# zwu88/TANTE

Measured on AMD Instinct MI355X. Metric: rollout frames/sec (fwd), TANTE on 256x256 Active Matter, higher is better.
Workload: dtype bf16

## Files before the change

### tante_amd/_lib.py

```python
import ctypes as C
import os

HERE = os.path.dirname(os.path.abspath(__file__))
LIB_PATH = os.environ.get("TANTE_LIB") or os.path.join(HERE, "lib", "libtante_hip.so")

F32, BF16 = 0, 1
ACT_NONE, ACT_GELU_ERF, ACT_GELU_TANH, ACT_RELU = 0, 1, 2, 3
A_LINEAR, A_PATCH_NHWC, A_PATCH_NCHW = 0, 1, 2
E_LINEAR, E_FILM, E_DECONV_NHWC, E_DECONV_NCHW = 0, 1, 2, 3
W_LINEAR, W_CONV_NHWC, W_DECONV_NHWC, W_DECONV_NCHW = 0, 1, 2, 3
W_LINEAR_T, W_CONV_NHWC_T, W_DECONV_NHWC_T, W_DECONV_NCHW_T = 4, 5, 6, 7

c_i32, c_i64, c_f32, c_vp = C.c_int32, C.c_int64, C.c_float, C.c_void_p


class PackGeom(C.Structure):
    _fields_ = [("n_pad", c_i32), ("k_pad", c_i32), ("nt", c_i32), ("cb", c_i32), ("bytes", c_i64)]


class Gemm(C.Structure):
    _fields_ = [
        ("a", c_vp), ("a_dtype", c_i32), ("a_mode", c_i32), ("M", c_i32), ("K", c_i32),
        ("a_s1", c_i64), ("a_s0", c_i64), ("a_off", c_i64), ("a_n0", c_i32),
        ("Hin", c_i32), ("Win", c_i32), ("Cin", c_i32), ("P", c_i32), ("ln", c_i32), ("ln_eps", c_f32),
# ... 160 lines not shown
    "tante_layernorm_bwd": ([c_vp, c_i32, c_vp, c_vp, c_vp, c_i64, c_i32, c_vp, c_vp], c_i32),
    "tante_act_fwd": ([c_vp, c_i32, c_vp, c_i32, c_i64, c_i32, c_vp], c_i32),
    "tante_act_bwd": ([c_vp, c_i32, c_vp, c_i32, c_vp, c_i32, c_i64, c_i32, c_vp], c_i32),
    "tante_colsum": ([c_vp, c_i32, c_i64, c_i32, c_i64, c_vp, c_i32, c_vp], c_i32),
    "tante_film_pos_fwd": ([c_vp, c_vp, c_vp, c_vp, c_i64, c_i32, c_i32, c_i64, c_vp, c_vp], c_i32),
    "tante_pos_embed_tmajor": ([c_vp, c_vp, c_vp, c_i64, c_i32, c_i64, c_i32, c_vp, c_vp], c_i32),
    "tante_film_pos_bwd": ([c_vp, c_vp, c_vp, c_i64, c_i64, c_i32, c_i32, c_vp, c_vp, c_vp, c_vp, c_vp], c_i32),
    "tante_taylor_bwd": ([c_vp, c_i64, C.POINTER(c_vp), c_i32, C.c_double, c_i32, c_vp, c_i64, c_i32, c_i64, c_i64, c_vp], c_i32),
    "tante_attention_bwd": ([c_vp, c_vp, c_vp, c_i32, c_i32, c_i32, C.POINTER(Seq), c_i32, c_f32, C.c_uint64, c_vp], c_i32),
    "tante_attention_dropout": ([c_vp, c_vp, c_i32, c_i32, c_i32, C.POINTER(Seq), c_i32, c_f32, C.c_uint64, c_vp], c_i32),
    "tante_dropout_add": ([c_vp, c_i32, c_vp, c_f32, C.c_uint64, c_i64, c_vp, c_vp], c_i32),
    "tante_dropout_bwd": ([c_vp, c_f32, C.c_uint64, c_i64, c_vp, c_i32, c_vp], c_i32),
    "tante_axis_mlp_bwd": ([c_vp, c_vp, c_i64, c_i32, c_i64, c_vp, c_vp, c_vp, c_vp, c_vp, c_vp, c_vp], c_i32),
    "tante_fold_fwd": ([c_vp, c_vp, c_vp, c_vp, c_i32, c_i32, c_vp, c_vp, c_vp], c_i32),
    "tante_fold_bwd": ([c_vp, c_vp, c_vp, c_vp, c_vp, c_i32, c_i32, c_vp, c_vp, c_vp, c_vp, c_vp], c_i32),
    "tante_fold_bwd_clear": ([c_vp, c_vp, c_vp, c_vp, c_vp, c_i32, c_i32, c_vp, c_vp, c_vp, c_vp, c_vp], c_i32),
    "tante_fold_bwd_multi": ([c_vp, c_i32, c_i32, c_vp], c_i32),
    "tante_fold_fwd_multi": ([c_vp, c_i32, c_vp], c_i32),
    "tante_axis_mlp_film_supported": ([c_i64, c_i32, c_i32, c_i64, c_i32], c_i32),
    "tante_axis_mlp_film": ([c_vp, c_vp, c_vp, c_vp, c_vp, c_i64, c_i32, c_i32, c_i64, c_i32, c_vp, c_vp, c_vp, c_vp, c_vp], c_i32),
    "tante_film_pos_fwd_frames": ([c_vp, c_vp, c_vp, c_vp, c_i64, c_i32, c_i64, c_i32, c_vp, c_vp], c_i32),
    "tante_film_pos_bwd_frames": ([c_vp, c_vp, c_vp, c_i64, c_i64, c_i32, c_i32, c_vp, c_vp, c_vp, c_vp, c_vp], c_i32),
    "tante_film_pos_bwd_frames_acc": ([c_vp, c_vp, c_vp, c_i64, c_i64, c_i32, c_i32, c_vp, c_i32, c_vp, c_vp, c_vp, c_i32, c_vp], c_i32),
    "tante_film_table_bwd": ([c_vp, c_i32, c_i32] + [c_vp] * 6 + [c_vp, c_vp] + [c_vp] * 8 + [c_i32, c_vp], c_i32),
    "tante_pack_block_train_multi": ([c_vp, c_i32, c_i32, c_i32, c_vp], c_i32),
    "tante_pack_block_tail_bwd_multi": ([c_vp, c_i32, c_i32, c_i32, c_vp], c_i32),
    "tante_axis_mlp_bwd_fused_supported": ([c_i32, c_i64], c_i32),
    "tante_axis_mlp_bwd_fused": ([c_vp, c_vp, c_i64, c_i32, c_i64, c_vp, c_vp, c_vp, c_vp, c_vp, c_vp, c_vp, c_vp, c_vp], c_i32),
    "tante_axis_mlp_bwd_fused_ws": ([c_vp, c_vp, c_i64, c_i32, c_i64, c_vp, c_vp, c_vp, c_vp, c_vp, c_vp, c_vp, c_vp, c_vp, c_i64, c_vp], c_i32),
    "tante_axis_wgrad": ([c_vp, c_vp, c_i64, c_i32, c_i64, c_vp, c_vp, c_i32, c_vp], c_i32),
    "tante_axis_wgrad_workspace_bytes": ([], c_i64),
    "tante_set_seed_mix": ([c_vp], c_i32),
    "tante_axis_wgrad_ws": ([c_vp, c_vp, c_i64, c_i32, c_i64, c_vp, c_vp, c_i32, c_vp, c_i64, c_vp], c_i32),
    "tante_wgrad": ([C.POINTER(RowMat), C.POINTER(RowMat), c_i64, c_i32, c_i32, c_vp, c_vp, c_i32, c_i32, c_i32, c_i32, c_i32, c_i32, c_vp], c_i32),
    "tante_wgrad_ws": ([C.POINTER(RowMat), C.POINTER(RowMat), c_i64, c_i32, c_i32, c_vp, c_vp, c_i32, c_i32, c_i32, c_i32, c_i32, c_i32, c_vp, c_i64, c_vp], c_i32),
    "tante_wgrad_multi_ws": ([c_vp, c_vp, c_i32, c_i64, c_i32, c_i32, c_vp, c_vp, c_i32, c_i32, c_i32, c_i32, c_i32, c_i32, c_vp, c_i64, c_vp], c_i32),
    "tante_wgrad_multi": ([c_vp, c_vp, c_i32, c_i64, c_i32, c_i32, c_vp, c_vp, c_i32, c_i32, c_i32, c_i32, c_i32, c_i32, c_vp], c_i32),
    "tante_clip_value": ([c_vp, c_i64, c_f32, c_vp], c_i32),
    "tante_rt_reduce_bwd": ([c_vp, c_i32, c_i32, c_vp, c_vp], c_i32),
    "tante_last_error": ([], C.c_char_p),
    "tante_abi_version": ([], c_i32),
    "tante_set_option": ([C.c_char_p, c_i32], c_i32),
    "tante_nan_to_num": ([c_vp, c_vp, c_i64, c_vp], c_i32),
    "tante_head_fused_multi": ([c_i32, c_vp, c_vp, c_vp, c_i32, c_i64, c_i64, c_i64, c_i32, c_i32, c_i32, c_i32, c_i32, c_vp, c_i64, c_vp, c_i64,
                               c_vp], c_i32),
    "tante_head_fused_multi_streams": ([c_i32, c_vp, c_vp, c_vp, c_i32, c_i64, c_i64, c_i64, c_i32, c_i32, c_i32, c_i32, c_i32, c_vp, c_i64, c_vp, c_i64,
                               c_vp], c_i32),
    "tante_spectral_bf16out_supported": ([c_i64, c_i32, c_i32, c_i32, c_i32, c_i32, c_i32], c_i32),
    "tante_spectral_layer_bf16out": ([c_vp, c_i64, c_i32, c_i32, c_i32, c_vp, c_vp, c_i32, c_i32, c_i32, c_i32, c_vp, c_vp, c_i32, c_i32, c_vp, c_vp,
                                     c_i64, c_vp], c_i32),
    "tante_get_option": ([C.c_char_p, c_i32], c_i32),
    "tante_attention_masked": ([c_vp, c_vp, c_i32, c_i32, c_i32, c_i32, c_i32, c_i32, c_vp, c_i64, c_vp, c_vp], c_i32),
    "tante_attention_masked_bwd": ([c_vp, c_vp, c_vp, c_i32, c_i32, c_i32, c_i32, c_i32, c_i32, c_vp, c_i64, c_vp, c_vp, c_vp], c_i32),
    "tante_attention_flash_stats_floats": ([c_i32, C.POINTER(Seq)], c_i64),
    "tante_attention_flash_supported": ([c_i32, c_i32, c_i32, c_i32], c_i32),
    "tante_attention_flash": ([c_vp, c_vp, c_vp, c_i32, c_i32, c_i32, C.POINTER(Seq), c_i32, c_f32, C.c_uint64, c_vp], c_i32),
    "tante_attention_flash_bwd": ([c_vp, c_vp, c_vp, c_vp, c_vp, c_i32, c_i32, c_i32, C.POINTER(Seq), c_i32, c_f32, C.c_uint64, c_vp], c_i32),
    "tante_attention_flash_masked": ([c_vp, c_vp, c_vp, c_i32, c_i32, c_i32, c_i32, c_i32, c_i32, c_vp, c_i64, c_vp, c_f32, C.c_uint64, c_vp], c_i32),
    "tante_attention_flash_masked_bwd": ([c_vp, c_vp, c_vp, c_vp, c_vp, c_i32, c_i32, c_i32, c_i32, c_i32, c_i32, c_vp, c_i64, c_vp, c_f32, C.c_uint64, c_vp], c_i32),
    "tante_head_enc_supported": ([c_i32, c_i32], c_i32),
    "tante_head_enc_stream_bytes": ([c_i32], c_i64),
    "tante_head_enc_ws_bytes": ([c_i64], c_i64),
    "tante_pack_head_enc": ([c_vp] * 6 + [c_i32, c_i32, c_vp, c_vp], c_i32),
    "tante_head_enc_fused": ([c_i32, c_vp, c_vp, c_vp, c_i32, c_i64, c_i64, c_i64, c_i32, c_i32, c_i32, c_i32, c_i32, c_vp, c_i64, c_vp, c_i64,
                             c_vp, c_vp, c_vp, c_i64, c_vp], c_i32),
    "tante_adaptive_tail_supported": ([c_i32] * 6, c_i32),
    "tante_adaptive_rt_stream_bytes": ([c_i32], c_i64),
    "tante_adaptive_ws_bytes": ([c_i32, c_i32, c_i32, c_i32], c_i64),
    "tante_pack_adaptive_rt": ([c_vp] * 6 + [c_i32, c_vp, c_vp], c_i32),
    "tante_adaptive_rt": ([c_i32, c_vp, c_vp, c_vp, c_i32, c_i64, c_i64, c_i64, c_i32, c_i32, c_i32, c_i32, c_f32, c_f32, c_vp, c_i64,
                           c_vp, c_vp, c_vp, c_vp, c_vp, c_vp], c_i32),
    "tante_head_adaptive": ([c_i32, c_vp, c_vp, c_i32, c_i64, c_i64, c_i64, c_i32, c_i32, c_i32, c_i32, c_i32, c_vp, c_vp, c_vp, c_i32, c_vp,
                             c_i32, c_vp, c_i64, c_vp, c_i64, c_vp], c_i32),
    "tante_afno_filter_supported": ([c_i64, c_i32, c_i32, c_i32, c_i32], c_i32),
    "tante_afno_twiddle_floats": ([c_i32, c_i32], c_i64),
    "tante_afno_filter_workspace_bytes": ([c_i64, c_i32, c_i32, c_i32], c_i64),
    "tante_afno_filter": ([c_vp, c_vp, c_i64, c_i32, c_i32, c_i32, c_i32, c_vp, c_vp, c_vp, c_f32, c_vp, c_vp, c_i64, c_vp], c_i32),
}

LIB_OPTIONS = ("TANTE_ATTN_BWD_HG", "TANTE_ATTN_BWD_NO_SPLIT", "TANTE_ATTN_BWD_VALU", "TANTE_ATTN_FWD_VALU", "TANTE_AXIS_BWD_SMALL_WGS",
               "TANTE_AXIS_BLOCKS", "TANTE_AXIS_BWD_WGS", "TANTE_AXIS_CT", "TANTE_AXIS_FILM", "TANTE_AXIS_GENERIC", "TANTE_AXIS_MFMA", "TANTE_AXIS_NT", "TANTE_AXIS_WGRAD_WGS",
               "TANTE_BLOCK_KERNEL", "TANTE_COLSUM_ROWS", "TANTE_CVIT_CHAIN_TOKENS", "TANTE_ENC23_SPLIT", "TANTE_FILM_BWD_ROWS",
               "TANTE_FS_GROUPS", "TANTE_FS_HALF", "TANTE_FS_SKEW", "TANTE_FS_WAVES", "TANTE_GEMM_NO_LITE", "TANTE_GEMM_SMALLM", "TANTE_GEMM_WGS", "TANTE_HEAD_WAVES",
               "TANTE_IM2COL_TILED", "TANTE_RESIZE_TILED", "TANTE_SPECTRAL_BF16OUT", "TANTE_SPECTRAL_DFT", "TANTE_SPECTRAL_X3", "TANTE_WGRAD_DEEP",
               "TANTE_WGRAD_JOBS", "TANTE_WGRAD_JOBS_WGS", "TANTE_WGRAD_NO_SLAB", "TANTE_WGRAD_NO_TR", "TANTE_WGRAD_REDUCE_NY",
               "TANTE_WGRAD_RG", "TANTE_WGRAD_SLAB_WGS", "TANTE_WGRAD_TR_WGS", "TANTE_WGRAD_WGS", "TANTE_XATTN_GPW", "TANTE_XATTN_STREAM", "TANTE_XATTN_VALU",)


_lib = None
ABI_VERSION = 14


def lib():
    global _lib
    if _lib is None:
        if not os.path.exists(LIB_PATH):
            raise RuntimeError(
                f"{LIB_PATH} is missing: build it with `python -m tante_amd.build` "
                "(or __graft_entry__.build()).  tante_amd has no CPU / eager fallback.")
        L = C.CDLL(LIB_PATH)
        for name, (argtypes, restype) in SIGNATURES.items():
            fn = getattr(L, name)
            fn.argtypes = argtypes
            fn.restype = restype
        got = int(L.tante_abi_version())
        if got != ABI_VERSION:
            raise RuntimeError(f"{LIB_PATH}: library ABI {got}, this binding expects {ABI_VERSION} -- a stale build (or a stale variant under "
                               "TANTE_LIB); rebuild with `python -m tante_amd.build`")
        _lib = L
        import warnings
        for k in LIB_OPTIONS:
            v = os.environ.get(k)
            if v is None:
                continue
            try:
                rc = L.tante_set_option(k.encode(), int(v))
            except ValueError:
                warnings.warn(f"{k}={v!r}: library options are integers; ignored")
                continue
            if rc != 0:
                warnings.warn(f"{k}={v}: tante_set_option refused it ({L.tante_last_error().decode(errors='replace')})")
    return _lib


def set_option(name: str, value: int) -> None:
    check(lib().tante_set_option(name.encode(), int(value)), "tante_set_option")


def get_option(name: str, default: int = 0) -> int:
    return int(lib().tante_get_option(name.encode(), int(default)))


def check(rc: int, what: str = ""):
    if rc != 0:
        msg = lib().tante_last_error().decode(errors="replace")
        raise RuntimeError(f"libtante_hip {what} failed (rc={rc}): {msg}")
```

### tante_amd/csrc/block_sliced.hip

```cpp
#include "common.hip.h"
#include "fused_common.hip.h"
#include "fs_common.hip.h"
#include "block_sliced.h"

namespace {


struct FsArgs {
  float* x;
  const char* w;
  TanteSeq sq;
  int causal;
  float eps;
  int spw;
  unsigned magic;
  float* out;
  unsigned short *xh1, *qkv, *o, *xh2, *hpre, *act;
  float *st1, *x1, *st2;
  float p_drop;
  unsigned long long seed_attn, seed_out, seed_mlp;
  const unsigned long long* seed_mix;
  unsigned long long* stamps;
  const float* tprop;
  int skew;
};

#ifdef TANTE_ABLATE
#define FS_STAMP(k)                                                                                        \
  do {                                                                                                     \
    if (A.stamps) {                                                                                        \
      unsigned long long t_;                                                                               \
      __builtin_amdgcn_sched_barrier(0);                                                                   \
      asm volatile("s_memtime %0\n\ts_waitcnt lgkmcnt(0)" : "=s"(t_)::"memory");                          \
      __builtin_amdgcn_sched_barrier(0);                                                                   \
      if (lane == 0) A.stamps[((long)vblock * 8 + wave) * 20 + (k)] = t_;                               \
    }                                                                                                      \
  } while (0)
unsigned long long* g_fs_stamps = nullptr;
#else
#define FS_STAMP(k)
#endif

__device__ __forceinline__ void fs_divmod(int a, int n, float rn, int& q, int& r) {
  q = (int)((float)a * rn);
  r = a - q * n;
  if (r >= n) { ++q; r -= n; }
  if (r < 0) { --q; r += n; }
}
struct FsSeqMap {
  float rs0, rl0;
  __device__ __forceinline__ explicit FsSeqMap(const TanteSeq& q) : rs0(__builtin_amdgcn_rcpf((float)q.n_s0)), rl0(__builtin_amdgcn_rcpf((float)q.n_l0)) {}
  __device__ __forceinline__ long token(const TanteSeq& q, int s, int l) const {
    int a, b, c, d;
    fs_divmod(s, q.n_s0, rs0, a, b);
    fs_divmod(l, q.n_l0, rl0, c, d);
    return (long)a * q.S1 + (long)b * q.S0 + (long)c * q.P1 + (long)d * q.P0;
  }
};


struct TpropW {
  float w1c[4], w2c[4];
  f32x4 b1v, b2v;
};
__device__ __forceinline__ void tprop_weights(const float* __restrict__ tp, int lane, TpropW& w) {
#pragma unroll
  for (int a = 0; a < 4; ++a) { w.w1c[a] = tp[4 * (lane & 3) + a]; w.w2c[a] = tp[20 + 4 * (lane & 3) + a]; }
  w.b1v = f32x4{tp[16], tp[17], tp[18], tp[19]};
  w.b2v = f32x4{tp[36], tp[37], tp[38], tp[39]};
}
__device__ __forceinline__ void tprop_apply(const TpropW& w, f32x4 (&xs)[4]) {
  f32x4 hid[4], yy[4];
#pragma unroll
  for (int e = 0; e < 4; ++e) {
    f32x4 h = w.b1v;
#pragma unroll
    for (int a = 0; a < 4; ++a) h = __builtin_amdgcn_mfma_f32_4x4x1f32(w.w1c[a], xs[a][e], h, 0, 0, 0);
    hid[e] = h;
  }
#pragma unroll
  for (int e = 0; e < 4; ++e) hid[e] = gelu_poly4<false>(hid[e]);
#pragma unroll
  for (int e = 0; e < 4; ++e) {
    f32x4 acc = f32x4{xs[0][e], xs[1][e], xs[2][e], xs[3][e]} + w.b2v;
#pragma unroll
    for (int j = 0; j < 4; ++j) acc = __builtin_amdgcn_mfma_f32_4x4x1f32(w.w2c[j], hid[e][j], acc, 0, 0, 0);
    yy[e] = acc;
  }
#pragma unroll
  for (int t = 0; t < 4; ++t) xs[t] = f32x4{yy[0][t], yy[1][t], yy[2][t], yy[3][t]};
}

constexpr int fs_group(int ntt, int nk) {
  int g = 1;
  for (int d = 1; d <= ntt; ++d)
    if (ntt % d == 0 && d * nk <= 8) g = d;
  return g;
}

template <int TPS, int NTT, int NW, bool TRAIN, int G = 1, bool TPROP = false, bool LASTQ = false>
__global__ __launch_bounds__(64 * NW * G, 2) void block_fs_kernel(FsArgs A) {
  static_assert(!TPROP || (TPS == 1 && !TRAIN), "the fused temporal propagator: T letter (L = 4), inference");
  static_assert(!LASTQ || (TPS == 1 && NW == 4 && G == 1 && !TRAIN), "the last-slot form: T letter (L = 4), 4 waves, inference");
  static_assert(G == 1 || (G == 2 && NW == 4), "the paired form is two 4-wave groups");
  constexpr int RT = 16 / NW;
  constexpr int HPW = RT / 2;
  constexpr int FS_PF8 = 3, FS_PF4 = 2;
  constexpr bool TIGHT = (NW == 4 && NTT == 4 && (TRAIN || TPS == 0)) || (NW == 8 && NTT == 8);
  constexpr int PF = (NW == 8 ? FS_PF8 : FS_PF4) - (TIGHT ? 1 : 0);
  constexpr int IMG = 16 * NTT * FS_ROW;
  constexpr int LDS_G = 2 * IMG + 16 * NTT * NW * 8 + FS_BIAS_FLOATS * 4;
  extern __shared__ __attribute__((aligned(16))) char smem_all[];
  const int grp = G == 1 ? 0 : __builtin_amdgcn_readfirstlane((int)threadIdx.x >> 8);
  char* const smem = smem_all + grp * LDS_G;
  char* const bufA = smem;
  char* const bufB = smem + IMG;
  char* const stat = smem + 2 * IMG;
  float* const lbias = (float*)(stat + 16 * NTT * NW * 8);
  const int tid = threadIdx.x & (64 * NW - 1), lane = tid & 63, kk = lane >> 4, l15 = lane & 15;
  const int wave = __builtin_amdgcn_readfirstlane(tid >> 6);
  const int vblock = (int)blockIdx.x * G + grp;
  if constexpr (G == 2) {
    if (grp == 1) __builtin_amdgcn_s_barrier();
  }
  if constexpr (G == 1) {
    if ((__builtin_amdgcn_s_getreg(0x1804) & 1u) == 1u) __builtin_amdgcn_s_setprio(3);
  }
  if constexpr (!TRAIN && G == 1) {
    if (A.skew > 0 && blockIdx.x >= (gridDim.x >> 1)) {
      for (int i = 0; i < A.skew; ++i) __builtin_amdgcn_s_sleep(8);
    }
  }
  float* const x = A.x;
  const unsigned long long smix = (TRAIN && A.seed_mix) ? *A.seed_mix : 0ull;
  const unsigned long long sd_attn = A.seed_attn ^ smix;
  const int L = A.sq.L;
  const int seq0 = vblock * A.spw;
  const int nlive = min(A.spw, A.sq.nseq - seq0) * L;
  const int nslot = A.spw * L;

  const FsW wq = fs_wstream(A.w, (unsigned)((RT * wave) * FS_FRAG + lane * 16));
  u32x4 wb[PF + 1][RT];
  FS_STAMP(0);
#ifdef TANTE_ABLATE
  if (A.stamps && lane == 0) {
    A.stamps[((long)vblock * 8 + wave) * 20 + 16] = __builtin_amdgcn_s_getreg((31 << 11) | 4);
    A.stamps[((long)vblock * 8 + wave) * 20 + 17] = __builtin_amdgcn_s_getreg((31 << 11) | 20);
    A.stamps[((long)vblock * 8 + wave) * 20 + 18] = __builtin_amdgcn_s_memrealtime();
  }
#endif
  int tslot[2];
  {
    const FsSeqMap smap(A.sq);
#pragma unroll
    for (int h = 0; h < (16 * NTT > 64 ? 2 : 1); ++h) {
      const int slot = lane + 64 * h;
      const int s = (int)(((unsigned)slot * A.magic) >> 16), p = slot - s * L;
      tslot[h] = slot < nlive ? (int)smap.token(A.sq, seq0 + s, p) : -1;
    }
  }
  auto tok_of = [&](int slot) { return __shfl(slot < 64 ? tslot[0] : tslot[16 * NTT > 64 ? 1 : 0], slot & 63); };
  for (int i = tid; i < FS_BIAS_FLOATS / 4; i += 64 * NW) *(f32x4*)(lbias + 4 * i) = *(const f32x4*)((const float*)(A.w + FS_W_BYTES) + 4 * i);
  FS_STAMP(1);
  int tokidx[NTT];
#pragma unroll
  for (int tt = 0; tt < NTT; ++tt) tokidx[tt] = tok_of(16 * tt + l15);

  constexpr int CPR = 4 * RT, RPI = 64 / CPR, ROWB = CPR * 16, TILEB = 16 * ROWB;
  constexpr int NSUB = (IMG / NW) / TILEB >= 2 ? 2 : 1;
  static_assert((IMG / NW) >= TILEB, "staging piece too small");
  char* const stg = bufA + wave * (IMG / NW);
  const int rrow = lane / CPR, rchunk = lane % CPR;
  auto srow = [&](int j) { return RPI * j + rrow; };
  auto slice_load = [&](const float* __restrict__ src, f32x4 (&raw)[NTT][RT]) {
#pragma unroll
    for (int tt = 0; tt < NTT; ++tt)
#pragma unroll
      for (int j = 0; j < RT; ++j) {
        const int t = tok_of(16 * tt + srow(j));
        raw[tt][j] = *(const f32x4*)(src + (long)(t < 0 ? 0 : t) * FS_C + 16 * RT * wave + 4 * rchunk);
      }
  };
  auto slice_to_acc = [&](const f32x4 (&raw)[NTT][RT], f32x4 (&acc)[RT][NTT]) {
#pragma unroll
    for (int tt = 0; tt < NTT; ++tt) {
      char* sb = stg + (tt % NSUB) * TILEB;
#pragma unroll
// ... 46 lines not shown
          xv[i][t] = *(const f32x4*)(x + (long)(tk < 0 ? 0 : tk) * FS_C + 4 * lane);
        }
      fs_wring_prime<0, RT, PF>(wq, wb);
      TpropW tw;
      tprop_weights(A.tprop, lane, tw);
#pragma unroll
      for (int i = 0; i < GPW; ++i) {
        tprop_apply(tw, xv[i]);
#pragma unroll
        for (int t = 0; t < 4; ++t) {
          const f32x4 y = xv[i][t];
          const int tk = tok_of(4 * (wave * GPW + i) + t);
          const bool live = tk >= 0;
          if (live && (!LASTQ || t == 3)) *(f32x4*)(x + (long)tk * FS_C + 4 * lane) = y;
          float sm = (y[0] + y[1]) + (y[2] + y[3]);
          float sq = fmaf(y[0], y[0], fmaf(y[1], y[1], fmaf(y[2], y[2], y[3] * y[3])));
          sm = rows_sum(row16_sum(sm));
          sq = rows_sum(row16_sum(sq));
          const float mean = sm * (1.0f / FS_C);
          const float var = fmaxf(sq * (1.0f / FS_C) - mean * mean, 0.0f);
          const float rstd = live ? rsqrtf(var + A.eps) : 0.0f;
          const float sh = live ? -mean * rstd : 0.0f;
          const int slot = 4 * (wave * GPW + i) + t;
          u32x2 o2;
          o2[0] = pack_bf16x2(fmaf(y[0], rstd, sh), fmaf(y[1], rstd, sh));
          o2[1] = pack_bf16x2(fmaf(y[2], rstd, sh), fmaf(y[3], rstd, sh));
          *(u32x2*)(bufA + slot * FS_ROW + (((lane >> 1) ^ (slot & 15)) << 4) + (lane & 1) * 8) = o2;
        }
      }
    }
  }
  if constexpr (!ln1_done) {
    constexpr int GPW = 4 * NTT / NW;
    static_assert(GPW * NW == 4 * NTT, "token rows must split evenly over the waves");
    f32x4 v[GPW][4];
    bool lv[GPW];
    int tis[GPW];
#pragma unroll
    for (int i = 0; i < GPW; ++i) {
      const int ti = tis[i] = tok_of(4 * (wave * GPW + i) + kk);
      lv[i] = ti >= 0;
      const float* row = x + (long)(lv[i] ? ti : 0) * FS_C;
#pragma unroll
      for (int j = 0; j < 4; ++j) v[i][j] = *(const f32x4*)(row + 4 * (l15 + 16 * j));
    }
    fs_wring_prime<0, RT, PF>(wq, wb);
#pragma unroll
    for (int i = 0; i < GPW; ++i) {
      float s = 0.f, q = 0.f;
#pragma unroll
      for (int j = 0; j < 4; ++j)
#pragma unroll
        for (int e = 0; e < 4; ++e) {
          s += v[i][j][e];
          q = fmaf(v[i][j][e], v[i][j][e], q);
        }
      s = row16_sum(s);
      q = row16_sum(q);
      const float mean = s * (1.0f / FS_C);
      const float var = fmaxf(q * (1.0f / FS_C) - mean * mean, 0.0f);
      const float rstd = lv[i] ? rsqrtf(var + A.eps) : 0.0f;
      const float sh = lv[i] ? -mean * rstd : 0.0f;
      const int slot = 4 * (wave * GPW + i) + kk, t15 = slot & 15;
#pragma unroll
      for (int j = 0; j < 4; ++j) {
        u32x2 o2;
        o2[0] = pack_bf16x2(fmaf(v[i][j][0], rstd, sh), fmaf(v[i][j][1], rstd, sh));
        o2[1] = pack_bf16x2(fmaf(v[i][j][2], rstd, sh), fmaf(v[i][j][3], rstd, sh));
        const int chunk = (l15 >> 1) + 8 * j;
        *(u32x2*)(bufA + slot * FS_ROW + ((chunk ^ t15) << 4) + (l15 & 1) * 8) = o2;
        if constexpr (TRAIN) {
          if (lv[i]) *(u32x2*)(A.xh1 + (long)tis[i] * FS_C + 4 * (l15 + 16 * j)) = o2;
        }
      }
      if constexpr (TRAIN) {
        if (lv[i] && l15 == 0) *(float2*)(A.st1 + 2 * (long)tis[i]) = make_float2(mean, rstd);
      }
    }
  }

  int rdo[4];
#pragma unroll
  for (int j = 0; j < 4; ++j) rdo[j] = l15 * FS_ROW + ((((j ^ (l15 >> 2)) << 2) | (kk ^ (l15 & 3))) << 4);
  int wro[RT];
#pragma unroll
  for (int rt = 0; rt < RT; ++rt) wro[rt] = l15 * FS_ROW + (((2 * RT * wave + 2 * rt + (kk >> 1)) ^ l15) << 4) + (kk & 1) * 8;

  const float* const bias = lbias + 16 * RT * wave + 4 * kk;

  FS_STAMP(2);
  __syncthreads();
  FS_STAMP(3);

  const f32x4 zero4 = f32x4{0.f, 0.f, 0.f, 0.f};
  constexpr int NP = (NTT + 1) / 2;
  u32x4 qf[HPW][NTT], kf[HPW][NTT];
  u32x4 vtf[HPW][2][NP];
  {
    f32x4 aq[RT][NTT];
#pragma unroll
    for (int j = 0; j < RT; ++j) {
      const f32x4 bq = *(const f32x4*)(bias + 16 * j);
#pragma unroll
      for (int tt = 0; tt < NTT; ++tt) aq[j][tt] = bq;
    }
    fs_slice_gemm<0, 24, NTT, RT, false, PF>(wq, wb, bufA, rdo, aq);
#pragma unroll
    for (int hh = 0; hh < HPW; ++hh)
#pragma unroll
      for (int tt = 0; tt < NTT; ++tt) qf[hh][tt] = pack8(aq[2 * hh][tt], aq[2 * hh + 1][tt]);
    if (TRAIN && A.qkv) {
      const float unscale = 1.0f / (0.17677669529663687f * 1.44269504088896340736f);
#pragma unroll
      for (int tt = 0; tt < NTT; ++tt) {
#pragma unroll
        for (int j = 0; j < RT; ++j) {
          const f32x4 qv = aq[j][tt] * unscale;
          u32x2 u;
          u[0] = pack_bf16x2(qv[0], qv[1]); u[1] = pack_bf16x2(qv[2], qv[3]);
          *(u32x2*)(bufB + tt * 8192 + wro[j]) = u;
        }
        img_rows_store(bufB, tt, A.qkv, 3 * FS_C, 0);
      }
    }
  }
  FS_STAMP(4);
  {
    f32x4 ak[RT][NTT];
#pragma unroll
    for (int j = 0; j < RT; ++j) {
      const f32x4 bk = TRAIN ? *(const f32x4*)(bias + 1024 + 16 * j) : zero4;
#pragma unroll
      for (int tt = 0; tt < NTT; ++tt) ak[j][tt] = bk;
    }
    fs_slice_gemm<1, 24, NTT, RT, false, PF>(wq, wb, bufA, rdo, ak);
#pragma unroll
    for (int hh = 0; hh < HPW; ++hh)
#pragma unroll
      for (int tt = 0; tt < NTT; ++tt) kf[hh][tt] = pack8(ak[2 * hh][tt], ak[2 * hh + 1][tt]);
    if (TRAIN && A.qkv) {
#pragma unroll
      for (int tt = 0; tt < NTT; ++tt) {
#pragma unroll
        for (int j = 0; j < RT; ++j) {
          u32x2 u;
          u[0] = pack_bf16x2(ak[j][tt][0], ak[j][tt][1]); u[1] = pack_bf16x2(ak[j][tt][2], ak[j][tt][3]);
          *(u32x2*)(bufB + tt * 8192 + wro[j]) = u;
        }
        img_rows_store(bufB, tt, A.qkv, 3 * FS_C, FS_C);
      }
    }
  }
  FS_STAMP(5);
  {
    f32x4 av[RT][NTT];
#pragma unroll
    for (int j = 0; j < RT; ++j) {
      const float bv = TRAIN ? lbias[1280 + 16 * RT * wave + 16 * j + l15] : 0.0f;
#pragma unroll
      for (int tt = 0; tt < NTT; ++tt) av[j][tt] = f32x4{bv, bv, bv, bv};
    }
    fs_slice_gemm<2, 24, NTT, RT, true, PF>(wq, wb, bufA, rdo, av);
    if (TRAIN && A.qkv) {
#pragma unroll
      for (int tt = 0; tt < NTT; ++tt) {
#pragma unroll
        for (int r = 0; r < 4; ++r) {
          const int row = 4 * kk + r;
#pragma unroll
          for (int j = 0; j < RT; ++j) {
            const __bf16 b = (__bf16)av[j][tt][r];
            *(unsigned short*)(bufB + tt * 8192 + row * FS_ROW + (((CPB * wave + 2 * j + (l15 >> 3)) ^ row) << 4) + (l15 & 7) * 2) =
                __builtin_bit_cast(unsigned short, b);
          }
        }
        img_rows_store(bufB, tt, A.qkv, 3 * FS_C, 2 * FS_C);
      }
    }
#pragma unroll
    for (int hh = 0; hh < HPW; ++hh)
#pragma unroll
      for (int p = 0; p < NP; ++p)
#pragma unroll
        for (int dt = 0; dt < 2; ++dt)
          vtf[hh][dt][p] = (2 * p + 1 < NTT) ? pack8(av[2 * hh + dt][2 * p], av[2 * hh + dt][2 * p + 1]) : pack8(av[2 * hh + dt][2 * p], zero4);
  }
  FS_STAMP(6);
  if constexpr (G == 2) __builtin_amdgcn_s_barrier();

  {
    unsigned allow1 = 0xfu;
    bool nomask = true;
    if constexpr (TPS == 1) {
      allow1 = 0u;
      const int si = (int)(((unsigned)l15 * A.magic) >> 16), pi = l15 - si * L;
#pragma unroll
      for (int r = 0; r < 4; ++r) {
        const int j = 4 * kk + r, sj = (int)(((unsigned)j * A.magic) >> 16), pj = j - sj * L;
        allow1 |= ((sj == si && (!A.causal || pj <= pi)) ? 1u : 0u) << r;
      }
      nomask = (L == 16) && !A.causal;
    }
    constexpr int NK = TPS > 0 ? TPS : NTT;
    constexpr int QG = fs_group(NTT, NK);
    static_for<HPW * (NTT / QG)>([&](auto hg_c) {
      constexpr int hh = decltype(hg_c)::value / (NTT / QG), q0 = (decltype(hg_c)::value % (NTT / QG)) * QG;
      f32x4 sc[QG][NK];
      unsigned allow[QG];
      float mx[QG], sum[QG];
      static_for<QG>([&](auto qt_c) {
        constexpr int q = decltype(qt_c)::value, qt = q0 + q;
        constexpr int k0 = TPS > 0 ? (qt / TPS) * TPS : 0;
#pragma unroll
        for (int j = 0; j < NK; ++j) sc[q][j] = mfma_bf16(kf[hh][k0 + j], qf[hh][qt], zero4);
      });
#pragma unroll
      for (int qt = 0; qt < QG; ++qt) {
        if constexpr (TPS == 0) {
          const int qs = 16 * (q0 + qt) + l15, si = (int)(((unsigned)qs * A.magic) >> 16), pi = qs - si * L;
          allow[qt] = 0u;
#pragma unroll
          for (int j = 0; j < NK; ++j)
#pragma unroll
            for (int r = 0; r < 4; ++r) {
              const int ksl = 16 * j + 4 * kk + r, sj = (int)(((unsigned)ksl * A.magic) >> 16), pj = ksl - sj * L;
              allow[qt] |= ((sj == si && ksl < nslot && (!A.causal || pj <= pi)) ? 1u : 0u) << (4 * j + r);
            }
        } else {
          allow[qt] = allow1 * 0x11111111u;
        }
      }
      if (TPS != 0 && nomask) {
#pragma unroll
        for (int qt = 0; qt < QG; ++qt) {
          float m = -INFINITY;
#pragma unroll
          for (int j = 0; j < NK; ++j) m = fmaxf(m, fmaxf(fmaxf(sc[qt][j][0], sc[qt][j][1]), fmaxf(sc[qt][j][2], sc[qt][j][3])));
          mx[qt] = m;
        }
      } else {
#pragma unroll
        for (int qt = 0; qt < QG; ++qt) {
          float m = -INFINITY;
#pragma unroll
          for (int j = 0; j < NK; ++j)
#pragma unroll
            for (int r = 0; r < 4; ++r)
              if ((allow[qt] >> (4 * j + r)) & 1u) m = fmaxf(m, sc[qt][j][r]);
          mx[qt] = m;
        }
      }
#pragma unroll
      for (int qt = 0; qt < QG; ++qt) mx[qt] = rows_max(mx[qt]);
      if (TPS != 0 && nomask) {
#pragma unroll
        for (int qt = 0; qt < QG; ++qt) {
          float sm = 0.0f;
#pragma unroll
          for (int j = 0; j < NK; ++j)
#pragma unroll
            for (int r = 0; r < 4; ++r) {
              sc[qt][j][r] = __builtin_amdgcn_exp2f(sc[qt][j][r] - mx[qt]);
              sm += sc[qt][j][r];
            }
          sum[qt] = sm;
        }
      } else {
#pragma unroll
        for (int qt = 0; qt < QG; ++qt) {
          float sm = 0.0f;
#pragma unroll
          for (int j = 0; j < NK; ++j)
#pragma unroll
            for (int r = 0; r < 4; ++r) {
              sc[qt][j][r] = ((allow[qt] >> (4 * j + r)) & 1u) ? __builtin_amdgcn_exp2f(sc[qt][j][r] - mx[qt]) : 0.0f;
              sm += sc[qt][j][r];
            }
          sum[qt] = sm;
        }
      }
#pragma unroll
      for (int qt = 0; qt < QG; ++qt) sum[qt] = rows_sum(sum[qt]);
      if constexpr (TRAIN) {
        if (A.p_drop > 0.0f) {
          const float ksc = 1.0f / (1.0f - A.p_drop);
          static_for<QG>([&](auto qt_c) {
            constexpr int qt = decltype(qt_c)::value;
            constexpr int k0 = TPS > 0 ? ((q0 + qt) / TPS) * TPS : 0;
            const int qs = 16 * (q0 + qt) + l15, si = (int)(((unsigned)qs * A.magic) >> 16), pi = qs - si * L;
            const unsigned long long mrow = ((((unsigned long long)(seq0 + si)) * 8 + (HPW * wave + hh)) * L + pi) * L;
#pragma unroll
            for (int j = 0; j < NK; ++j) {
              const int jpos0 = 16 * (k0 + j) + 4 * kk - si * L;
              if ((L & 3) == 0) {
                const unsigned m4 = dropout_keep4(sd_attn, mrow + (unsigned long long)(jpos0 < 0 ? 0 : jpos0), A.p_drop);
#pragma unroll
                for (int r = 0; r < 4; ++r) sc[qt][j][r] = ((m4 >> r) & 1u) ? sc[qt][j][r] * ksc : 0.0f;
              } else {
#pragma unroll
                for (int r = 0; r < 4; ++r) {
                  const int jpos = jpos0 + r;
                  sc[qt][j][r] = dropout_keep(sd_attn, mrow + (unsigned long long)(jpos < 0 ? 0 : jpos), A.p_drop) ? sc[qt][j][r] * ksc : 0.0f;
                }
              }
            }
          });
        }
      }
      f32x4 o[QG][2];
      static_for<QG>([&](auto qt_c) {
        constexpr int qt = decltype(qt_c)::value;
        constexpr int k0 = TPS > 0 ? ((q0 + qt) / TPS) * TPS : 0;
        constexpr int g0 = k0 / 2, g1 = (k0 + NK - 1) / 2;
        o[qt][0] = o[qt][1] = zero4;
        static_for<g1 - g0 + 1>([&](auto g_c) {
          constexpr int g = g0 + decltype(g_c)::value;
          constexpr int ja = 2 * g - k0, jb = 2 * g + 1 - k0;
          f32x4 pa = zero4, pb = zero4;
          if constexpr (ja >= 0 && ja < NK) pa = sc[qt][ja];
          if constexpr (jb >= 0 && jb < NK) pb = sc[qt][jb];
          const u32x4 pf = pack8(pa, pb);
          o[qt][0] = mfma_bf16(vtf[hh][0][g], pf, o[qt][0]);
          o[qt][1] = mfma_bf16(vtf[hh][1][g], pf, o[qt][1]);
        });
      });
#pragma unroll
      for (int qt = 0; qt < QG; ++qt) {
        const float inv = sum[qt] > 0.0f ? __builtin_amdgcn_rcpf(sum[qt]) : 0.0f;
        const f32x4 o0 = o[qt][0] * inv, o1 = o[qt][1] * inv;
        u32x2 w0, w1;
        w0[0] = pack_bf16x2(o0[0], o0[1]); w0[1] = pack_bf16x2(o0[2], o0[3]);
        w1[0] = pack_bf16x2(o1[0], o1[1]); w1[1] = pack_bf16x2(o1[2], o1[3]);
        *(u32x2*)(bufB + (q0 + qt) * 8192 + wro[2 * hh]) = w0;
        *(u32x2*)(bufB + (q0 + qt) * 8192 + wro[2 * hh + 1]) = w1;
      }
    });
  }
  if constexpr (TRAIN) {
#pragma unroll
    for (int tt = 0; tt < NTT; ++tt) img_rows_store(bufB, tt, A.o, FS_C, 0);
  }

  FS_STAMP(7);
  asm volatile("" ::: "memory");
  f32x4 xraw[NTT][RT];
  fs_wring_prime<3, RT, PF>(wq, wb);
  slice_load(x, xraw);
  FS_STAMP(8);
  __syncthreads();
  FS_STAMP(9);

  f32x4 x1[RT][NTT];
#pragma unroll
  for (int rt = 0; rt < RT; ++rt) {
    const f32x4 bo = *(const f32x4*)(bias + (TRAIN ? 1536 : 256) + 16 * rt);
#pragma unroll
    for (int tt = 0; tt < NTT; ++tt) x1[rt][tt] = bo;
  }
  fs_slice_gemm<3, 48, NTT, RT, false, PF>(wq, wb, bufB, rdo, x1);
  auto drop_add = [&](f32x4 (&acc)[RT][NTT], f32x4 (&res)[RT][NTT], unsigned long long seed) {
    if constexpr (TRAIN) {
      if (A.p_drop > 0.0f) {
        const float ksc = 1.0f / (1.0f - A.p_drop);
#pragma unroll
        for (int tt = 0; tt < NTT; ++tt) {
          const unsigned long long i0 = (unsigned long long)(tokidx[tt] < 0 ? 0 : tokidx[tt]) * FS_C + 16 * RT * wave + 4 * kk;
#pragma unroll
          for (int rt = 0; rt < RT; ++rt) {
            const unsigned k01 = dropout_keep2(seed, i0 + 16 * rt, A.p_drop), k23 = dropout_keep2(seed, i0 + 16 * rt + 2, A.p_drop);
            acc[rt][tt][0] = (k01 & 1u) ? acc[rt][tt][0] * ksc : 0.0f;
            acc[rt][tt][1] = (k01 & 2u) ? acc[rt][tt][1] * ksc : 0.0f;
            acc[rt][tt][2] = (k23 & 1u) ? acc[rt][tt][2] * ksc : 0.0f;
            acc[rt][tt][3] = (k23 & 2u) ? acc[rt][tt][3] * ksc : 0.0f;
          }
        }
      }
    }
#pragma unroll
    for (int rt = 0; rt < RT; ++rt)
#pragma unroll
      for (int tt = 0; tt < NTT; ++tt) acc[rt][tt] += res[rt][tt];
  };
  {
    f32x4 xr[RT][NTT];
    slice_to_acc(xraw, xr);
    drop_add(x1, xr, A.seed_out ^ smix);
  }
  if constexpr (TRAIN) {
    if (A.x1) slice_store(A.x1, x1);
  }
  FS_STAMP(10);
#pragma unroll
  for (int tt = 0; tt < NTT; ++tt) {
    float s = 0.f, q = 0.f;
#pragma unroll
    for (int rt = 0; rt < RT; ++rt)
#pragma unroll
      for (int r = 0; r < 4; ++r) {
        s += x1[rt][tt][r];
        q = fmaf(x1[rt][tt][r], x1[rt][tt][r], q);
      }
    s = rows_sum(s);
    q = rows_sum(q);
    if (kk == 0) *(float2*)(stat + ((16 * tt + l15) * NW + wave) * 8) = make_float2(s, q);
  }
  __syncthreads();
  FS_STAMP(11);
#pragma unroll
  for (int tt = 0; tt < NTT; ++tt) {
    const f32x4* sp = (const f32x4*)(stat + (16 * tt + l15) * NW * 8);
    float s = 0.f, q = 0.f;
#pragma unroll
    for (int j = 0; j < NW / 2; ++j) {
      const f32x4 a = sp[j];
      s += a[0] + a[2];
      q += a[1] + a[3];
    }
    const float mean = s * (1.0f / FS_C);
    const float var = fmaxf(q * (1.0f / FS_C) - mean * mean, 0.0f);
    const float rstd = rsqrtf(var + A.eps);
    const float sh = -mean * rstd;
#pragma unroll
    for (int rt = 0; rt < RT; ++rt) {
      u32x2 o2;
      o2[0] = pack_bf16x2(fmaf(x1[rt][tt][0], rstd, sh), fmaf(x1[rt][tt][1], rstd, sh));
      o2[1] = pack_bf16x2(fmaf(x1[rt][tt][2], rstd, sh), fmaf(x1[rt][tt][3], rstd, sh));
// ... 89 lines not shown
  const int nfrag = FS_W_BYTES / FS_FRAG;
  if (bid < nfrag / 4) {
    const int f = bid * 4 + (threadIdx.x >> 6), lane = threadIdx.x & 63, l15 = lane & 15, kk = lane >> 4;
    const int g = f % 16, ks = (f / 16) % 8, m = f / 128;
    const int row = (m < 3 ? m * C : 0) + 16 * g + l15;
    const float* src = m < 3 ? w_in : (m == 3 ? w_out : (m == 4 ? w1 : w2));
    const float* gamma = m < 3 ? g1 : (m == 4 ? g2 : nullptr);
    const float scale = m == 0 ? qscale : 1.0f;
    float v[8];
#pragma unroll
    for (int e = 0; e < 8; ++e) {
      const int k = 32 * ks + 8 * kk + e;
      float xv = src[(long)row * C + k];
      if (gamma) xv *= gamma[k];
      v[e] = xv * scale;
    }
    u32x4 o;
    o[0] = pack_bf16x2(v[0], v[1]); o[1] = pack_bf16x2(v[2], v[3]); o[2] = pack_bf16x2(v[4], v[5]); o[3] = pack_bf16x2(v[6], v[7]);
    *(u32x4*)(dst + (long)f * FS_FRAG + lane * 16) = o;
    return;
  }
  __shared__ float bv[FS_C];
  const int n = threadIdx.x;
  if (!be1) {
    float* bias = (float*)(dst + FS_W_BYTES);
    bias[n] = b_in[n] * qscale;
    bias[256 + n] = b_out[n];
    bias[512 + n] = b1[n];
    bias[768 + n] = b2[n];
    bias[1024 + n] = b_in[C + n];
    bias[1280 + n] = b_in[2 * C + n];
    bias[1536 + n] = b_out[n];
    return;
  }
  {
    float s = b_in[2 * C + n];
    for (int k = 0; k < C; ++k) s += w_in[(long)(2 * C + n) * C + k] * be1[k];
    bv[n] = s;
  }
  __syncthreads();
  float* bias = (float*)(dst + FS_W_BYTES);
  {
    float s = b_in[n];
    for (int k = 0; k < C; ++k) s += w_in[(long)n * C + k] * be1[k];
    bias[n] = s * qscale;
  }
  {
    float s = b_out[n];
    for (int c = 0; c < C; ++c) s += w_out[(long)n * C + c] * bv[c];
    bias[256 + n] = s;
  }
  {
    float s = b1[n];
    for (int k = 0; k < C; ++k) s += w1[(long)n * C + k] * be2[k];
    bias[512 + n] = s;
  }
  bias[768 + n] = b2[n];
  {
    float s = b_in[C + n];
    for (int k = 0; k < C; ++k) s += w_in[(long)(C + n) * C + k] * be1[k];
    bias[1024 + n] = s;
  }
  bias[1280 + n] = bv[n];
  bias[1536 + n] = b_out[n];
}
__global__ void fs_pack_kernel(const float* __restrict__ w_in, const float* __restrict__ b_in, const float* __restrict__ g1,
                               const float* __restrict__ be1, const float* __restrict__ w_out, const float* __restrict__ b_out,
                               const float* __restrict__ w1, const float* __restrict__ b1, const float* __restrict__ g2,
                               const float* __restrict__ be2, const float* __restrict__ w2, const float* __restrict__ b2,
                               char* __restrict__ dst) {
  fs_pack_body((int)blockIdx.x, w_in, b_in, g1, be1, w_out, b_out, w1, b1, g2, be2, w2, b2, dst);
}
constexpr int FSP_BLOCKS = FS_W_BYTES / FS_FRAG / 4 + 1;
struct FsPackBatch {
  const float* p[TANTE_FSP_MAX][8];
  char* dst[TANTE_FSP_MAX];
};
__global__ void fs_pack_multi_kernel(FsPackBatch B) {
  const int e = blockIdx.x / FSP_BLOCKS;
  const float* const* q = B.p[e];
  fs_pack_body((int)blockIdx.x - e * FSP_BLOCKS, q[0], q[1], nullptr, nullptr, q[2], q[3], q[4], q[5], nullptr, nullptr, q[6], q[7], B.dst[e]);
}

template <int TPS, int NTT, int NW, bool TRAIN, int G = 1, bool TPROP = false, bool LASTQ = false>
void fs_launch_tt(const FsArgs& A, int nwg, hipStream_t s) {
  constexpr int LDS = G * (2 * 16 * NTT * FS_ROW + 16 * NTT * NW * 8 + FS_BIAS_FLOATS * 4);
  static_assert(LDS <= 160 * 1024, "LDS per workgroup");
  static TantePerDevice attr;
  attr.once([&] { (void)hipFuncSetAttribute((const void*)block_fs_kernel<TPS, NTT, NW, TRAIN, G, TPROP, LASTQ>, hipFuncAttributeMaxDynamicSharedMemorySize, LDS); });
  hipLaunchKernelGGL((block_fs_kernel<TPS, NTT, NW, TRAIN, G, TPROP, LASTQ>), dim3((nwg + G - 1) / G), dim3(64 * NW * G), LDS, s, A);
}
template <int NTT>
void fs_launch_last(const FsArgs& A, int nwg, hipStream_t s) {
  if (A.tprop) fs_launch_tt<1, NTT, 4, false, 1, true, true>(A, nwg, s);
  else fs_launch_tt<1, NTT, 4, false, 1, false, true>(A, nwg, s);
}
template <int TPS, int NTT, int NW>
void fs_launch_t(const FsArgs& A, int nwg, hipStream_t s) {
  if constexpr (NW == 4) {
    if (A.out) return fs_launch_tt<TPS, NTT, NW, true>(A, nwg, s);
    if constexpr (TPS == 1) {
      if (A.tprop) return fs_launch_tt<TPS, NTT, NW, false, 1, true>(A, nwg, s);
    }
    const int groups = tante_opt("TANTE_FS_GROUPS", 0);
    if (groups == 2) return fs_launch_tt<TPS, NTT, NW, false, 2>(A, nwg, s);
  }
  fs_launch_tt<TPS, NTT, NW, false>(A, nwg, s);
}

int fs_waves(int L) {
  const int force8 = tante_opt("TANTE_FS_WAVES", 0) == 8;
  return (force8 || L > 64) ? 8 : 4;
}

}

#ifdef TANTE_ABLATE
extern "C" void tante_fs_set_stamps(void* p) { g_fs_stamps = (unsigned long long*)p; }
#endif

int tante_fs_supported(int C, int n_head, int hidden, int L, int causal) {
  (void)causal;
  return C == FS_C && n_head == 8 && hidden == FS_C && L >= 1 && L <= 128;
}

int64_t tante_fs_stream_bytes(int C, int hidden) { return (C == FS_C && hidden == FS_C) ? FS_W_BYTES + FS_BIAS_FLOATS * 4 : 0; }

void tante_fs_pack(const float* ln1_w, const float* ln1_b, const float* in_w, const float* in_b, const float* out_w, const float* out_b,
                   const float* ln2_w, const float* ln2_b, const float* fc1_w, const float* fc1_b, const float* fc2_w,
                   const float* fc2_b, char* dst, hipStream_t s) {
  hipLaunchKernelGGL(fs_pack_kernel, dim3(FS_W_BYTES / FS_FRAG / 4 + 1), dim3(256), 0, s, in_w, in_b, ln1_w, ln1_b, out_w, out_b, fc1_w,
                     fc1_b, ln2_w, ln2_b, fc2_w, fc2_b, dst);
}

void tante_fs_pack_folded(const float* in_w, const float* in_b, const float* out_w, const float* out_b, const float* fc1_w,
                          const float* fc1_b, const float* fc2_w, const float* fc2_b, char* dst, hipStream_t s) {
  hipLaunchKernelGGL(fs_pack_kernel, dim3(FS_W_BYTES / FS_FRAG / 4 + 1), dim3(256), 0, s, in_w, in_b, (const float*)nullptr,
                     (const float*)nullptr, out_w, out_b, fc1_w, fc1_b, (const float*)nullptr, (const float*)nullptr, fc2_w, fc2_b, dst);
}

void tante_fs_pack_folded_multi(const float* const (*params)[8], char* const* dst, int n, hipStream_t s) {
  FsPackBatch B;
  for (int e = 0; e < n; ++e) {
    for (int k = 0; k < 8; ++k) B.p[e][k] = params[e][k];
    B.dst[e] = dst[e];
  }
  hipLaunchKernelGGL(fs_pack_multi_kernel, dim3((unsigned)(n * FSP_BLOCKS)), dim3(256), 0, s, B);
}

int tante_fs_launch(float* x, const char* stream, const TanteSeq& sq, int causal, float eps, hipStream_t s, const TanteBlockTrain* tr,
                    const float* tprop, bool lastq) {
  if (sq.nseq >= (1 << 23)) return -2;
  if (tprop && (tr || sq.L != 4)) return -5;
  if (lastq && (tr || sq.L != 4)) return -5;
  FsArgs A;
  A.x = x; A.w = stream; A.sq = sq; A.causal = causal; A.eps = eps;
  A.out = nullptr;
  A.seed_mix = nullptr;
  A.tprop = tprop;
  if (tr) {
    if (sq.L > 64) return -4;
    A.out = tr->out; A.xh1 = (unsigned short*)tr->xh1; A.st1 = tr->st1; A.qkv = (unsigned short*)tr->qkv; A.o = (unsigned short*)tr->o;
    A.x1 = tr->x1; A.xh2 = (unsigned short*)tr->xh2; A.st2 = tr->st2; A.hpre = (unsigned short*)tr->hpre; A.act = (unsigned short*)tr->act;
    A.p_drop = tr->p_drop; A.seed_attn = tr->seed_attn; A.seed_out = tr->seed_out; A.seed_mlp = tr->seed_mlp;
    A.seed_mix = tante_seed_mix_ptr();
  }
  A.stamps = nullptr;
#ifdef TANTE_ABLATE
  A.stamps = g_fs_stamps;
#endif
  const int L = sq.L, nw = (tr || tprop || lastq) ? 4 : fs_waves(L);
  A.magic = (65536u + (unsigned)L - 1u) / (unsigned)L;
  int tps = 0;
  if (16 % L == 0) tps = 1;
  else if (!causal && (L == 32 || L == 48 || L == 64)) tps = L / 16;
  const int full = nw == 8 ? 8 : 4, tq = nw == 8 ? 6 : 3;
  const long resident = 256L * (8 / nw);
  auto rounds = [&](int ntt) {
// ... 45 lines not shown
```

Before: 19090.

## Compute only last-slot query rows in the fused block's last-layer kernel

Adds a LASTQ=2 mode to the fused sliced block kernel, on by default through TANTE_LAST_QTILE. It gathers only the slot-(L-1) query rows into one tile, computes their attention against all keys, and runs the out-projection, LayerNorm and MLP on that single tile instead of every token tile. This removes the Q projection, attention output and MLP GEMM work for rows that are computed but never stored in the last-slot path. It adds a separate code path with its own gathered row indexing, and a mistake in that indexing could give wrong results.

New measurement: 19140 (median of 6 runs). About the same (+0.2%).

```diff
diff --git a/tante_amd/_lib.py b/tante_amd/_lib.py
--- a/tante_amd/_lib.py
+++ b/tante_amd/_lib.py
@@ -266,7 +266,7 @@
                "TANTE_AXIS_BLOCKS", "TANTE_AXIS_BWD_WGS", "TANTE_AXIS_CT", "TANTE_AXIS_FILM", "TANTE_AXIS_GENERIC", "TANTE_AXIS_MFMA", "TANTE_AXIS_NT", "TANTE_AXIS_WGRAD_WGS",
                "TANTE_BLOCK_KERNEL", "TANTE_COLSUM_ROWS", "TANTE_CVIT_CHAIN_TOKENS", "TANTE_ENC23_SPLIT", "TANTE_FILM_BWD_ROWS",
                "TANTE_FS_GROUPS", "TANTE_FS_HALF", "TANTE_FS_SKEW", "TANTE_FS_WAVES", "TANTE_GEMM_NO_LITE", "TANTE_GEMM_SMALLM", "TANTE_GEMM_WGS", "TANTE_HEAD_WAVES",
-               "TANTE_IM2COL_TILED", "TANTE_RESIZE_TILED", "TANTE_SPECTRAL_BF16OUT", "TANTE_SPECTRAL_DFT", "TANTE_SPECTRAL_X3", "TANTE_WGRAD_DEEP",
+               "TANTE_IM2COL_TILED", "TANTE_LAST_QTILE", "TANTE_RESIZE_TILED", "TANTE_SPECTRAL_BF16OUT", "TANTE_SPECTRAL_DFT", "TANTE_SPECTRAL_X3", "TANTE_WGRAD_DEEP",
                "TANTE_WGRAD_JOBS", "TANTE_WGRAD_JOBS_WGS", "TANTE_WGRAD_NO_SLAB", "TANTE_WGRAD_NO_TR", "TANTE_WGRAD_REDUCE_NY",
                "TANTE_WGRAD_RG", "TANTE_WGRAD_SLAB_WGS", "TANTE_WGRAD_TR_WGS", "TANTE_WGRAD_WGS", "TANTE_XATTN_GPW", "TANTE_XATTN_STREAM", "TANTE_XATTN_VALU",)
 
diff --git a/tante_amd/csrc/block_sliced.hip b/tante_amd/csrc/block_sliced.hip
--- a/tante_amd/csrc/block_sliced.hip
+++ b/tante_amd/csrc/block_sliced.hip
@@ -98,11 +98,14 @@
   return g;
 }
 
-template <int TPS, int NTT, int NW, bool TRAIN, int G = 1, bool TPROP = false, bool LASTQ = false>
+template <int TPS, int NTT, int NW, bool TRAIN, int G = 1, bool TPROP = false, int LASTQ = 0>
 __global__ __launch_bounds__(64 * NW * G, 2) void block_fs_kernel(FsArgs A) {
   static_assert(!TPROP || (TPS == 1 && !TRAIN), "the fused temporal propagator: T letter (L = 4), inference");
   static_assert(!LASTQ || (TPS == 1 && NW == 4 && G == 1 && !TRAIN), "the last-slot form: T letter (L = 4), 4 waves, inference");
   static_assert(G == 1 || (G == 2 && NW == 4), "the paired form is two 4-wave groups");
+  static_assert(LASTQ >= 0 && LASTQ <= 2, "0 = every row, 1 = every row computed and the slot-(L - 1) rows stored, 2 = the query side on one gathered tile");
+  constexpr bool QT = LASTQ == 2;
+  constexpr int NTQ = QT ? 1 : NTT;
   constexpr int RT = 16 / NW;
   constexpr int HPW = RT / 2;
   constexpr int FS_PF8 = 3, FS_PF4 = 2;
@@ -315,6 +318,10 @@
   int rdo[4];
 #pragma unroll
   for (int j = 0; j < 4; ++j) rdo[j] = l15 * FS_ROW + ((((j ^ (l15 >> 2)) << 2) | (kk ^ (l15 & 3))) << 4);
+  int rdoq[4];
+#pragma unroll
+  for (int j = 0; j < 4; ++j)
+    rdoq[j] = ((l15 >> 2) & (NTT - 1)) * 8192 + (4 * (l15 & 3) + 3) * FS_ROW + ((((j ^ (l15 & 3)) << 2) | (kk ^ 3)) << 4);
   int wro[RT];
 #pragma unroll
   for (int rt = 0; rt < RT; ++rt) wro[rt] = l15 * FS_ROW + (((2 * RT * wave + 2 * rt + (kk >> 1)) ^ l15) << 4) + (kk & 1) * 8;
@@ -327,22 +334,22 @@
 
   const f32x4 zero4 = f32x4{0.f, 0.f, 0.f, 0.f};
   constexpr int NP = (NTT + 1) / 2;
-  u32x4 qf[HPW][NTT], kf[HPW][NTT];
+  u32x4 qf[HPW][NTQ], kf[HPW][NTT];
   u32x4 vtf[HPW][2][NP];
   {
-    f32x4 aq[RT][NTT];
+    f32x4 aq[RT][NTQ];
 #pragma unroll
     for (int j = 0; j < RT; ++j) {
       const f32x4 bq = *(const f32x4*)(bias + 16 * j);
 #pragma unroll
-      for (int tt = 0; tt < NTT; ++tt) aq[j][tt] = bq;
-    }
-    fs_slice_gemm<0, 24, NTT, RT, false, PF>(wq, wb, bufA, rdo, aq);
+      for (int tt = 0; tt < NTQ; ++tt) aq[j][tt] = bq;
+    }
+    fs_slice_gemm<0, 24, NTQ, RT, false, PF>(wq, wb, bufA, QT ? rdoq : rdo, aq);
 #pragma unroll
     for (int hh = 0; hh < HPW; ++hh)
 #pragma unroll
-      for (int tt = 0; tt < NTT; ++tt) qf[hh][tt] = pack8(aq[2 * hh][tt], aq[2 * hh + 1][tt]);
-    if (TRAIN && A.qkv) {
+      for (int tt = 0; tt < NTQ; ++tt) qf[hh][tt] = pack8(aq[2 * hh][tt], aq[2 * hh + 1][tt]);
+    if constexpr (TRAIN) if (A.qkv) {
       const float unscale = 1.0f / (0.17677669529663687f * 1.44269504088896340736f);
 #pragma unroll
       for (int tt = 0; tt < NTT; ++tt) {
@@ -421,7 +428,49 @@
   FS_STAMP(6);
   if constexpr (G == 2) __builtin_amdgcn_s_barrier();
 
-  {
+  if constexpr (QT) {
+    const int tq = l15 >> 2;
+    const bool mine = kk == (l15 & 3);
+#pragma unroll
+    for (int hh = 0; hh < HPW; ++hh) {
+      f32x4 s4 = mfma_bf16(kf[hh][0], qf[hh][0], zero4);
+#pragma unroll
+      for (int t = 1; t < NTT; ++t) {
+        const f32x4 st = mfma_bf16(kf[hh][t], qf[hh][0], zero4);
+#pragma unroll
+        for (int r = 0; r < 4; ++r) s4[r] = tq == t ? st[r] : s4[r];
+      }
+      float m = -INFINITY;
+#pragma unroll
+      for (int r = 0; r < 4; ++r) m = mine ? fmaxf(m, s4[r]) : m;
+      const float mx = rows_max(m);
+      f32x4 e;
+      float sm = 0.0f;
+#pragma unroll
+      for (int r = 0; r < 4; ++r) {
+        e[r] = mine ? __builtin_amdgcn_exp2f(s4[r] - mx) : 0.0f;
+        sm += e[r];
+      }
+      const float sum = rows_sum(sm);
+      f32x4 o0 = zero4, o1 = zero4;
+#pragma unroll
+      for (int g = 0; g < NP; ++g) {
+        const f32x4 pa = tq == 2 * g ? e : zero4, pb = tq == 2 * g + 1 ? e : zero4;
+        const u32x4 pf = pack8(pa, pb);
+        o0 = mfma_bf16(vtf[hh][0][g], pf, o0);
+        o1 = mfma_bf16(vtf[hh][1][g], pf, o1);
+      }
+      const float inv = sum > 0.0f ? __builtin_amdgcn_rcpf(sum) : 0.0f;
+      o0 = o0 * inv;
+      o1 = o1 * inv;
+      u32x2 w0, w1;
+      w0[0] = pack_bf16x2(o0[0], o0[1]); w0[1] = pack_bf16x2(o0[2], o0[3]);
+      w1[0] = pack_bf16x2(o1[0], o1[1]); w1[1] = pack_bf16x2(o1[2], o1[3]);
+      *(u32x2*)(bufB + wro[2 * hh]) = w0;
+      *(u32x2*)(bufB + wro[2 * hh + 1]) = w1;
+    }
+  }
+  if constexpr (!QT) {
     unsigned allow1 = 0xfu;
     bool nomask = true;
     if constexpr (TPS == 1) {
@@ -575,6 +624,102 @@
   }
 
   FS_STAMP(7);
+  if constexpr (QT) {
+    asm volatile("" ::: "memory");
+    fs_wring_prime<3, RT, PF>(wq, wb);
+    f32x4 xg[RT];
+#pragma unroll
+    for (int j = 0; j < RT; ++j) {
+      const int g = srow(j), t = tok_of(16 * (g >> 2) + 4 * (g & 3) + 3);
+      xg[j] = *(const f32x4*)(x + (long)(t < 0 ? 0 : t) * FS_C + 16 * RT * wave + 4 * rchunk);
+    }
+    FS_STAMP(8);
+    __syncthreads();
+    FS_STAMP(9);
+    f32x4 x1[RT][1];
+#pragma unroll
+    for (int rt = 0; rt < RT; ++rt) x1[rt][0] = *(const f32x4*)(bias + 256 + 16 * rt);
+    fs_slice_gemm<3, 48, 1, RT, false, PF>(wq, wb, bufB, rdo, x1);
+#pragma unroll
+    for (int j = 0; j < RT; ++j) {
+      const int r = srow(j);
+      *(f32x4*)(stg + r * ROWB + ((rchunk ^ (r & (CPR - 1))) << 4)) = xg[j];
+    }
+#pragma unroll
+    for (int rt = 0; rt < RT; ++rt) x1[rt][0] += *(const f32x4*)(stg + l15 * ROWB + (((4 * rt + kk) ^ (l15 & (CPR - 1))) << 4));
+    FS_STAMP(10);
+    {
+      float s = 0.f, q = 0.f;
+#pragma unroll
+      for (int rt = 0; rt < RT; ++rt)
+#pragma unroll
+        for (int r = 0; r < 4; ++r) {
+          s += x1[rt][0][r];
+          q = fmaf(x1[rt][0][r], x1[rt][0][r], q);
+        }
+      s = rows_sum(s);
+      q = rows_sum(q);
+      if (kk == 0) *(float2*)(stat + (l15 * NW + wave) * 8) = make_float2(s, q);
+    }
+    __syncthreads();
+    FS_STAMP(11);
+    {
+      const f32x4* sp = (const f32x4*)(stat + l15 * NW * 8);
+      float s = 0.f, q = 0.f;
+#pragma unroll
+      for (int j = 0; j < NW / 2; ++j) {
+        const f32x4 a = sp[j];
+        s += a[0] + a[2];
+        q += a[1] + a[3];
+      }
+      const float mean = s * (1.0f / FS_C);
+      const float var = fmaxf(q * (1.0f / FS_C) - mean * mean, 0.0f);
+      const float rstd = rsqrtf(var + A.eps);
+      const float sh = -mean * rstd;
+#pragma unroll
+      for (int rt = 0; rt < RT; ++rt) {
+        u32x2 o2;
+        o2[0] = pack_bf16x2(fmaf(x1[rt][0][0], rstd, sh), fmaf(x1[rt][0][1], rstd, sh));
+        o2[1] = pack_bf16x2(fmaf(x1[rt][0][2], rstd, sh), fmaf(x1[rt][0][3], rstd, sh));
+        *(u32x2*)(bufA + wro[rt]) = o2;
+      }
+    }
+    __syncthreads();
+    FS_STAMP(12);
+    {
+      f32x4 h[RT][1];
+#pragma unroll
+      for (int rt = 0; rt < RT; ++rt) h[rt][0] = *(const f32x4*)(bias + 512 + 16 * rt);
+      fs_slice_gemm<4, 48, 1, RT, false, PF>(wq, wb, bufA, rdo, h);
+      FS_STAMP(13);
+#pragma unroll
+      for (int rt = 0; rt < RT; ++rt) {
+        const f32x4 g = gelu_poly4<true>(h[rt][0]);
+        u32x2 o2;
+        o2[0] = pack_bf16x2(g[0], g[1]);
+        o2[1] = pack_bf16x2(g[2], g[3]);
+        *(u32x2*)(bufB + wro[rt]) = o2;
+      }
+    }
+    __syncthreads();
+    FS_STAMP(14);
+#pragma unroll
+    for (int rt = 0; rt < RT; ++rt) x1[rt][0] += *(const f32x4*)(bias + 768 + 16 * rt);
+    fs_slice_gemm<5, 48, 1, RT, false, PF>(wq, wb, bufB, rdo, x1);
+    FS_STAMP(15);
+#ifdef TANTE_ABLATE
+    if (A.stamps && lane == 0) A.stamps[((long)vblock * 8 + wave) * 20 + 19] = __builtin_amdgcn_s_memrealtime();
+#endif
+#pragma unroll
+    for (int rt = 0; rt < RT; ++rt) *(f32x4*)(stg + l15 * ROWB + (((4 * rt + kk) ^ (l15 & (CPR - 1))) << 4)) = x1[rt][0];
+#pragma unroll
+    for (int j = 0; j < RT; ++j) {
+      const int g = srow(j), t = tok_of(16 * (g >> 2) + 4 * (g & 3) + 3);
+      const f32x4 v = *(const f32x4*)(stg + g * ROWB + ((rchunk ^ (g & (CPR - 1))) << 4));
+      if (t >= 0) st_wt16(x + (long)t * FS_C + 16 * RT * wave + 4 * rchunk, v);
+    }
+    return;
+  }
   asm volatile("" ::: "memory");
   f32x4 xraw[NTT][RT];
   fs_wring_prime<3, RT, PF>(wq, wb);
@@ -830,7 +975,7 @@
   fs_pack_body((int)blockIdx.x - e * FSP_BLOCKS, q[0], q[1], nullptr, nullptr, q[2], q[3], q[4], q[5], nullptr, nullptr, q[6], q[7], B.dst[e]);
 }
 
-template <int TPS, int NTT, int NW, bool TRAIN, int G = 1, bool TPROP = false, bool LASTQ = false>
+template <int TPS, int NTT, int NW, bool TRAIN, int G = 1, bool TPROP = false, int LASTQ = 0>
 void fs_launch_tt(const FsArgs& A, int nwg, hipStream_t s) {
   constexpr int LDS = G * (2 * 16 * NTT * FS_ROW + 16 * NTT * NW * 8 + FS_BIAS_FLOATS * 4);
   static_assert(LDS <= 160 * 1024, "LDS per workgroup");
@@ -840,8 +985,13 @@
 }
 template <int NTT>
 void fs_launch_last(const FsArgs& A, int nwg, hipStream_t s) {
-  if (A.tprop) fs_launch_tt<1, NTT, 4, false, 1, true, true>(A, nwg, s);
-  else fs_launch_tt<1, NTT, 4, false, 1, false, true>(A, nwg, s);
+  if (tante_opt("TANTE_LAST_QTILE", 1)) {
+    if (A.tprop) fs_launch_tt<1, NTT, 4, false, 1, true, 2>(A, nwg, s);
+    else fs_launch_tt<1, NTT, 4, false, 1, false, 2>(A, nwg, s);
+  } else {
+    if (A.tprop) fs_launch_tt<1, NTT, 4, false, 1, true, 1>(A, nwg, s);
+    else fs_launch_tt<1, NTT, 4, false, 1, false, 1>(A, nwg, s);
+  }
 }
 template <int TPS, int NTT, int NW>
 void fs_launch_t(const FsArgs& A, int nwg, hipStream_t s) {
```
